# willis-richard/connect4

Measured on AMD Instinct MI355X. Metric: mcts_node_expansions_per_sec, higher is better.
Workload: dtype f32x3

## Files before the change

### connect4_amd/csrc/c4_engine.hip

```cpp
#include <hip/hip_runtime.h>
#include <hip/hip_fp16.h>
#include <hip/hip_bfloat16.h>

#include <algorithm>
#include <cmath>
#include <cstdarg>
#include <cstdio>
#include <cstdlib>
#include <cstring>
#include <limits>
#include <vector>

#include "../../include/c4_engine.h"
#include "c4_board.h"
#include "c4_net_dev.h"

#ifndef C4_DEADLINE_EVERY
#define C4_DEADLINE_EVERY 1
#endif
#ifndef C4_TERMQ
#define C4_TERMQ 1
#endif
#ifndef C4_FUSED_NET_STAMPS
#define C4_FUSED_NET_STAMPS 0
#endif
#ifndef C4_ASM_PICK
#define C4_ASM_PICK 1
#endif
#ifndef C4_SPECULATE
#define C4_SPECULATE 1
#endif
#ifndef C4_SPLIT_PHASES
#define C4_SPLIT_PHASES 0
#endif
#ifndef C4_DIV_NORMAL
#define C4_DIV_NORMAL 1
#endif
#ifndef C4_SCORE_ALL
#define C4_SCORE_ALL 1
#endif
#ifndef C4_PATH_ALL_LANES
#define C4_PATH_ALL_LANES 1
#endif
#ifndef C4_PEEL_BACKUP
#define C4_PEEL_BACKUP 1
#endif
#ifndef C4_NO_SUSPEND
#define C4_NO_SUSPEND 1
#endif
#ifndef C4_NET_SANITISES
#define C4_NET_SANITISES 1
#endif
#ifndef C4_WAIT_CLOCK_LAZY
#define C4_WAIT_CLOCK_LAZY 1
#endif
#ifndef C4_SPLIT_PAIRS
#define C4_SPLIT_PAIRS 1
#endif
#ifndef C4_SORT_SLOTS
#define C4_SORT_SLOTS 1
#endif
#ifndef C4_FILLERS
#define C4_FILLERS (C4_ORIENTED_Q && C4_SCORE_ALL)
#endif
#ifndef C4_VGPR_BASES
#define C4_VGPR_BASES 1
#endif
#ifndef C4_ORIENTED_Q
#define C4_ORIENTED_Q 1
#endif
#ifndef C4_COOP_LEGAL
#define C4_COOP_LEGAL 1
#endif
#ifndef C4_PICK_BPERM
#define C4_PICK_BPERM 1
#endif
#ifndef C4_EARLY_REQUEST
#define C4_EARLY_REQUEST 1
#endif

namespace {

using namespace c4;

constexpr int GROUP = 8;
constexpr int SLOTS_PER_BLOCK = 8;
constexpr int BLOCK = GROUP * SLOTS_PER_BLOCK;
constexpr int MAX_DEPTH = 44;

constexpr int SLOT_ACTIVE = 0;
constexpr int SLOT_PARKED = 1;
constexpr int SLOT_MOVE_DONE = 2;

__host__ __device__ __forceinline__ uint32_t pack_info(uint32_t base, uint32_t nchild, uint32_t status,
                                                       uint32_t bit, uint32_t pf64)
{
    return (base >> 3) | (nchild << 19) | (status << 22) | (bit << 25) | (pf64 << 31);
}
__host__ __device__ __forceinline__ uint32_t info_base(uint32_t i) { return (i & 0x7ffffu) << 3; }
__host__ __device__ __forceinline__ uint32_t info_nchild(uint32_t i) { return (i >> 19) & 7u; }
__host__ __device__ __forceinline__ uint32_t info_status(uint32_t i) { return (i >> 22) & 7u; }
__host__ __device__ __forceinline__ uint32_t info_bit(uint32_t i) { return (i >> 25) & 63u; }
__host__ __device__ __forceinline__ uint32_t info_move(uint32_t i) { return info_bit(i) / 7u; }
__host__ __device__ __forceinline__ uint32_t info_pf64(uint32_t i) { return i >> 31; }

struct __attribute__((aligned(16))) PathEntry {
    uint32_t node;
    uint32_t n;
    double w;
};

constexpr int BLOCK_BYTES = 256;
struct __attribute__((aligned(32))) Rec {
    double w;
    double q;
    double p;
// ... 112 lines not shown
__device__ __forceinline__ float lds_ldf(const float *p) { return *(lds_vf32_t *)p; }
__device__ __forceinline__ void lds_st64(uint64_t *p, uint64_t v) { *(lds_vu64_t *)p = v; }

__device__ __forceinline__ void group_fence()
{
    __builtin_amdgcn_fence(__ATOMIC_RELEASE, "workgroup");
    __builtin_amdgcn_fence(__ATOMIC_ACQUIRE, "workgroup");
}

__device__ __forceinline__ void philox_round(uint32_t c[4], const uint32_t k[2])
{
    const uint64_t p0 = (uint64_t)0xD2511F53u * c[0];
    const uint64_t p1 = (uint64_t)0xCD9E8D57u * c[2];
    const uint32_t n0 = (uint32_t)(p1 >> 32) ^ c[1] ^ k[0];
    const uint32_t n1 = (uint32_t)p1;
    const uint32_t n2 = (uint32_t)(p0 >> 32) ^ c[3] ^ k[1];
    const uint32_t n3 = (uint32_t)p0;
    c[0] = n0; c[1] = n1; c[2] = n2; c[3] = n3;
}
__device__ inline void philox4x32(uint32_t c[4], uint64_t seed)
{
    uint32_t k[2] = {(uint32_t)seed, (uint32_t)(seed >> 32)};
#pragma unroll
    for (int r = 0; r < 10; ++r) {
        philox_round(c, k);
        k[0] += 0x9E3779B9u;
        k[1] += 0xBB67AE85u;
    }
}
__device__ inline void rng_uniform2(uint64_t seed, long long gid, uint32_t ply, uint32_t stream, uint32_t idx,
                                    double &u0, double &u1)
{
    uint32_t c[4] = {(uint32_t)gid, (uint32_t)((uint64_t)gid >> 32), ply * 64u + stream, idx};
    philox4x32(c, seed);
    u0 = (double)((((uint64_t)c[0] << 32) | c[1]) >> 11) * (1.0 / 9007199254740992.0);
    u1 = (double)((((uint64_t)c[2] << 32) | c[3]) >> 11) * (1.0 / 9007199254740992.0);
}
__device__ inline double rng_gamma(uint64_t seed, long long gid, uint32_t ply, uint32_t stream, double alpha)
{
    double u0, u1;
    rng_uniform2(seed, gid, ply, stream, 0, u0, u1);
    double boost = 1.0;
    if (alpha < 1.0) {
        boost = pow(u0 > 0.0 ? u0 : 1e-300, 1.0 / alpha);
        alpha += 1.0;
    }
    const double dd = alpha - 1.0 / 3.0, cc = 1.0 / sqrt(9.0 * dd);
    for (uint32_t it = 1; it <= 24; ++it) {
        double a, b, uu, unused;
        rng_uniform2(seed, gid, ply, stream, 2 * it, a, b);
        rng_uniform2(seed, gid, ply, stream, 2 * it + 1, uu, unused);
        const double x = sqrt(-2.0 * log(a > 0.0 ? a : 1e-300)) * cos(6.283185307179586 * b);
        double v = 1.0 + cc * x;
        if (v <= 0.0) continue;
        v = v * v * v;
        if (uu < 1.0 - 0.0331 * x * x * x * x) return boost * dd * v;
        if (log(uu > 0.0 ? uu : 1e-300) < 0.5 * x * x + dd * (1.0 - v + log(v))) return boost * dd * v;
    }
    return boost * dd;
}

__device__ __forceinline__ double child_value_for(uint32_t status, uint32_t n, double q, int side)
{
    const bool term = status >= ST_XWIN;
#if C4_TERMQ
    const double v = q;
#else
    const double v = term ? 0.5 * (double)(status - ST_XWIN) : q;
#endif
    const double sv = side == 0 ? v : 1.0 - v;
    return (term || n > 0) ? sv : 0.0;
}

__device__ __forceinline__ double orient_q(double v, int parent_side)
{
#if C4_ORIENTED_Q
    return (parent_side & 1) ? 1.0 - v : v;
#else
    (void)parent_side;
    return v;
#endif
}

__device__ __forceinline__ double div_normal(double a, double b)
{
#if C4_DIV_NORMAL
    double r = __builtin_amdgcn_rcp(b);
    double e = __builtin_fma(-b, r, 1.0);
    r = __builtin_fma(r, e, r);
    e = __builtin_fma(-b, r, 1.0);
    r = __builtin_fma(r, e, r);
    const double q = a * r;
    const double rem = __builtin_fma(-b, q, a);
    return __builtin_fma(rem, r, q);
#else
    return a / b;
#endif
}

__device__ __forceinline__ double ucb_score(double A, double B, uint32_t nc, double p, double V, uint32_t pf64)
{
    const double pbc = A * div_normal(B, (double)(nc + 1));
    const double prior_score64 = pbc * p;
    const double s64 = prior_score64 + V;
    const float prior_score32 = (float)pbc * (float)p;
    const float s32 = prior_score32 + (float)V;
    return pf64 ? s64 : (double)s32;
}

__device__ __forceinline__ int legal_mask_group(uint64_t occ)
{
#if C4_COOP_LEGAL
    const int lane = (int)(threadIdx.x & (GROUP - 1));
    const bool legal = lane < WIDTH && col_count(occ, lane < WIDTH ? lane : 0) < HEIGHT;
    const unsigned long long b = __builtin_amdgcn_ballot_w64(legal);
    return (int)((b >> (threadIdx.x & 63u & ~(uint32_t)(GROUP - 1))) & 0x7fu);
#else
    return legal_mask(occ);
#endif
}

__device__ __forceinline__ int group_argmax(double s, int k)
{
#pragma unroll
    for (int m = 1; m < GROUP; m <<= 1) {
        const double os = __shfl_xor(s, m, GROUP);
        const int ok = __shfl_xor(k, m, GROUP);
        if (os > s || (os == s && ok > k)) { s = os; k = ok; }
    }
    return k;
}

template <int CTRL>
__device__ __forceinline__ uint32_t dpp_u32(uint32_t v)
{
    return (uint32_t)__builtin_amdgcn_update_dpp(0, (int)v, CTRL, 0xF, 0xF, true);
}
template <int CTRL>
__device__ __forceinline__ double dpp_f64(double v)
{
    const uint64_t b = (uint64_t)__double_as_longlong(v);
    const uint64_t r = ((uint64_t)dpp_u32<CTRL>((uint32_t)(b >> 32)) << 32) | dpp_u32<CTRL>((uint32_t)b);
    return __longlong_as_double((long long)r);
}
struct Pick {
    double s;
    int k;
    uint32_t n, info;
    double w;
};
#define C4_DPP_SELECT(CTRL)                                                                              \
    asm volatile("s_mov_b64 vcc, %[m]\n"                                                                 \
                 "s_nop 0\n"                                                                             \
                 "v_cndmask_b32_dpp %[n], %[n], %[n], vcc " CTRL " row_mask:0xf bank_mask:0xf\n"         \
                 "v_cndmask_b32_dpp %[i], %[i], %[i], vcc " CTRL " row_mask:0xf bank_mask:0xf\n"         \
                 "v_cndmask_b32_dpp %[wl], %[wl], %[wl], vcc " CTRL " row_mask:0xf bank_mask:0xf\n"      \
                 "v_cndmask_b32_dpp %[wh], %[wh], %[wh], vcc " CTRL " row_mask:0xf bank_mask:0xf\n"      \
                 : [n] "+v"(n), [i] "+v"(info), [wl] "+v"(wl), [wh] "+v"(wh)                              \
                 : [m] "s"(m)                                                                             \
                 : "vcc")
#if C4_ASM_PICK
#define C4_PICK_SELECT(CTRL)                                                                             \
    asm volatile("s_mov_b64 vcc, %[m]\n"                                                                 \
                 "s_nop 0\n"                                                                             \
                 "v_cndmask_b32 %[sl], %[ol], %[sl], vcc\n"                                               \
                 "v_cndmask_b32 %[sh], %[oh], %[sh], vcc\n"                                               \
                 "v_cndmask_b32_dpp %[n], %[n], %[n], vcc " CTRL " row_mask:0xf bank_mask:0xf\n"          \
                 "v_cndmask_b32_dpp %[i], %[i], %[i], vcc " CTRL " row_mask:0xf bank_mask:0xf\n"          \
                 "v_cndmask_b32_dpp %[wl], %[wl], %[wl], vcc " CTRL " row_mask:0xf bank_mask:0xf\n"       \
                 "v_cndmask_b32_dpp %[wh], %[wh], %[wh], vcc " CTRL " row_mask:0xf bank_mask:0xf\n"       \
                 : [sl] "+v"(sl), [sh] "+v"(sh), [n] "+v"(n), [i] "+v"(info), [wl] "+v"(wl), [wh] "+v"(wh) \
                 : [m] "s"(m), [ol] "v"(ol), [oh] "v"(oh)                                                   \
                 : "vcc")
template <int CTRL>
__device__ __forceinline__ void pick_step(double &s, uint32_t &n, uint32_t &info, uint32_t &wl, uint32_t &wh)
{
    const uint64_t sb = (uint64_t)__double_as_longlong(s);
    uint32_t sl = (uint32_t)sb, sh = (uint32_t)(sb >> 32);
    const uint32_t ol = dpp_u32<CTRL>(sl), oh = dpp_u32<CTRL>(sh);
    const double os = __longlong_as_double((long long)(((uint64_t)oh << 32) | ol));
    constexpr unsigned long long HIGH = CTRL == 0xB1 ? 0xAAAAAAAAAAAAAAAAull : (CTRL == 0x4E ? 0xCCCCCCCCCCCCCCCCull : 0xF0F0F0F0F0F0F0F0ull);
// ... 67 lines not shown
__device__ __forceinline__ double dirichlet_from_gamma(double nz, bool legal)
{
    if (!legal) nz = 0.0;
    double s = 0.0;
#pragma unroll
    for (int i = 0; i < 7; ++i) s = s + gshfl(nz, i);
    return nz / s;
}

__device__ __forceinline__ int sample_child_sq(double V, bool act, uint32_t nc, double u, int lane)
{
    const double w2 = act ? V * V : 0.0;
    double s2 = 0.0;
#pragma unroll
    for (int i = 0; i < 7; ++i) s2 = s2 + gshfl(w2, i);
    if (!(s2 > 0.0)) return -1;
    const double pk = w2 / s2;
    double acc = 0.0, cdf = 0.0;
#pragma unroll
    for (int i = 0; i < 7; ++i) {
        acc = acc + gshfl(pk, i);
        if (i == lane) cdf = acc;
    }
    const double last = gshfl(cdf, (int)nc - 1);
    cdf = cdf / last;
    const unsigned long long bal = __ballot(act && cdf <= u);
    const int cnt = __popcll((bal >> (((threadIdx.x & 63) / GROUP) * GROUP)) & 0xffull);
    return cnt < (int)nc ? cnt : (int)nc - 1;
}

template <class DevT>
__device__ __forceinline__ void publish_game(DevT &d, int g, long long gid, int len, int32_t result, int lane)
{
    group_fence();
    int ok = 0;
    unsigned long long t = 0;
    if (lane == 0) {
        const unsigned long long tail = *(volatile unsigned long long *)d.cold->ring_tail;
        unsigned long long old = *(volatile unsigned long long *)d.cold->ring_head;
        for (;;) {
            if (old - tail >= (unsigned long long)d.rec_cap) { atomicAdd(d.cold->dropped, 1ULL); break; }
            const unsigned long long seen = atomicCAS(d.cold->ring_head, old, old + 1);
            if (seen == old) { ok = 1; t = old; break; }
            old = seen;
        }
    }
    ok = gshfl(ok, 0);
    if (!ok) return;
    t = ((unsigned long long)gshfl((uint32_t)(t >> 32), 0) << 32) | gshfl((uint32_t)t, 0);
    c4_game_record *row = d.cold->ring + (size_t)(t % (unsigned long long)d.rec_cap);
    const size_t s0 = (size_t)g * 42;
    for (int i = lane; i < len; i += GROUP) {
        row->color0[i] = d.cold->stg_c0[s0 + i];
        row->color1[i] = d.cold->stg_c1[s0 + i];
        row->move[i] = d.cold->stg_move[s0 + i];
        row->value[i] = d.cold->stg_value[s0 + i];
    }
    double *rp = &row->policy[0][0];
    for (int i = lane; i < len * 7; i += GROUP) rp[i] = d.cold->stg_policy[s0 * 7 + i];
    if (lane == 0) { row->game_id = gid; row->length = len; row->result = result; }
}

__device__ __forceinline__ uint64_t group_xor64(uint64_t v)
{
    uint32_t lo = (uint32_t)v, hi = (uint32_t)(v >> 32);
    lo ^= dpp_u32<0xB1>(lo); hi ^= dpp_u32<0xB1>(hi);
    lo ^= dpp_u32<0x4E>(lo); hi ^= dpp_u32<0x4E>(hi);
    lo ^= dpp_u32<0x141>(lo); hi ^= dpp_u32<0x141>(hi);
    return ((uint64_t)hi << 32) | lo;
}
__device__ __forceinline__ uint64_t cache_key(uint64_t c0, uint64_t c1) { return c0 + (c0 | c1); }
template <class DevT>
__device__ __forceinline__ CacheEntry *cache_slot(DevT &d, uint64_t key)
{
    return d.cache + ((key * 0x9E3779B97F4A7C15ULL) >> (64 - d.cache_bits));
}
__device__ __forceinline__ uint64_t cache_check(uint64_t key, float value, float prior_lane, int lane)
{
    const uint32_t bits = lane < 7 ? __float_as_uint(prior_lane) : __float_as_uint(value);
    const uint64_t w = ((uint64_t)bits << 32) | (uint32_t)(bits * 0x9E3779B1u + (uint32_t)lane);
    const int r = (lane * 7 + 3) & 63;
    return key ^ group_xor64((w << r) | (w >> ((64 - r) & 63)));
}
template <class DevT>
__device__ __forceinline__ bool cache_probe(DevT &d, uint64_t c0, uint64_t c1, int lane, float &value, float &prior_lane)
{
    const uint64_t key = cache_key(c0, c1);
    const CacheEntry *e = cache_slot(d, key);
    const uint64_t k = e->key, chk = e->check;
    value = e->value;
    prior_lane = lane < 7 ? e->prior[lane] : 0.0f;
    return k == key && chk == cache_check(key, value, prior_lane, lane);
}
template <class DevT>
__device__ __forceinline__ void cache_insert(DevT &d, uint64_t c0, uint64_t c1, int lane, float value, float prior_lane)
{
    const uint64_t key = cache_key(c0, c1);
    CacheEntry *e = cache_slot(d, key);
    const uint64_t chk = cache_check(key, value, prior_lane, lane);
    if (lane < 7) e->prior[lane] = prior_lane;
    if (lane == 0) { e->value = value; e->check = chk; e->key = key; }
}

template <typename T>
__device__ __forceinline__ void store_plane(void *planes, size_t idx, float v);
template <> __device__ __forceinline__ void store_plane<float>(void *p, size_t i, float v) { ((float *)p)[i] = v; }
template <> __device__ __forceinline__ void store_plane<__half>(void *p, size_t i, float v) { ((__half *)p)[i] = __float2half(v); }
template <> __device__ __forceinline__ void store_plane<hip_bfloat16>(void *p, size_t i, float v) { ((hip_bfloat16 *)p)[i] = hip_bfloat16(v); }

constexpr uint32_t REQ_IDLE = 0, REQ_POSTED = 1, REQ_TAKEN = 2, REQ_ANSWERED = 3;
template <int EVAL, bool STAMPS = true, bool LDS_STATE = false, bool WAVE_SYNC = false, bool PATH_KEPT = false, class DevT = const Dev,
          bool SPLIT = false>
__device__ __forceinline__ void tree_step(DevT &d, const int g, const int lane, const int gl,
                                          PathEntry (*s_path)[MAX_DEPTH], Rec (*s_l1)[GROUP],
                                          const void *__restrict__ values_in,
                                          const void *__restrict__ priors_in, void *__restrict__ planes_out,
                                          uint64_t *leaf_out, SlotMem *sm = nullptr, const int ai_lds = 0,
                                          uint32_t *wg_stats = nullptr, const unsigned long long deadline = 0,
                                          uint32_t *req = nullptr, const int diag_stride = 0)
{
    (void)diag_stride;
    static_assert(!SPLIT || (WAVE_SYNC && LDS_STATE && PATH_KEPT), "the split kernel keeps slot states and paths in LDS");
    if (leaf_out && lane < 2) leaf_out[lane] = 0;
    if (g >= d.slot_hi) return;
    if (LDS_STATE) {
        if (sm->state() != SLOT_ACTIVE) {
            if (lane == 0) sm->flags = SlotMem::pack(sm->state(), 0, sm->need_root());
            return;
        }
    } else if (d.state[g] != SLOT_ACTIVE) {
        if (lane == 0) d.has_leaf[g] = 0;
        return;
    }
    constexpr bool SCORE_F32 = (EVAL == C4_EVAL_EXTERNAL_F32);
    const int ai = LDS_STATE ? ai_lds : g;

    const Pool pool{d.pool + (size_t)g * d.cap * (BLOCK_BYTES / 8)};
    PathEntry *gpath = d.path + (size_t)g * MAX_DEPTH;

    uint64_t root0, root1;
    uint32_t sims, nalloc, pdepth, pinfo, ply;
    int32_t pend, need_root;
    long long gid;
    if (LDS_STATE) {
        root0 = sm->root0; root1 = sm->root1;
        sims = sm->sims; nalloc = sm->nalloc; pend = sm->pend; pdepth = sm->pdepth; pinfo = sm->pinfo;
        need_root = sm->need_root(); ply = sm->ply; gid = sm->gid;
    } else {
        root0 = d.root_c0[g]; root1 = d.root_c1[g];
        sims = d.sims_done[g]; nalloc = d.n_alloc[g]; pend = d.pending[g]; pdepth = d.pending_depth[g];
        pinfo = d.pending_info[g]; need_root = d.need_root[g]; ply = d.ply[g]; gid = d.game_id[g];
    }
    double root_w = LDS_STATE ? sm->root_w : 0.0;
    int state = SLOT_ACTIVE;
    int has_leaf = 0;
    struct { uint32_t sims, expansions, children, terminal_sims, leaf_evals, depth_sum, moves, games_started,
                      games_finished, capped, cache_hits, cache_probes, bad_evals, spec_evals; } st = {};
    static_assert(sizeof(st) == N_STATS * 4, "launch-local stats mirror SlotStats");

    uint64_t leaf0 = 0, leaf1 = 0;
    double ev_value = 0.0, ev_prior = 0.0;
    bool apply_now = false;
    bool path_lds = (EVAL == C4_EVAL_CENTRE) || PATH_KEPT;
    bool fresh_eval = false;
    bool cached_answer = false;
    if (SPLIT && pend >= 0) {
        if (lds_ld(req) != REQ_ANSWERED) return;
        if (lane == 0) lds_st(req, REQ_IDLE);
    }
    if (pend >= 0) {
        leaf0 = LDS_STATE ? sm->leaf0 : d.leaf_c0[g];
        leaf1 = LDS_STATE ? sm->leaf1 : d.leaf_c1[g];
        if (EVAL == C4_EVAL_EXTERNAL_F32) {
            ev_value = (double)((const float *)values_in)[ai];
            ev_prior = lane < 7 ? (double)((const float *)priors_in)[(size_t)ai * 7 + lane] : 0.0;
        } else if (EVAL == C4_EVAL_EXTERNAL_F64) {
            ev_value = ((const double *)values_in)[ai];
            ev_prior = lane < 7 ? ((const double *)priors_in)[(size_t)ai * 7 + lane] : 0.0;
        }
        apply_now = true;
        fresh_eval = (EVAL == C4_EVAL_EXTERNAL_F32) && d.cache != nullptr;
    }

    auto stamp = [&](int i) {
        if (STAMPS && d.has_stamps && blockIdx.x < 256 && threadIdx.x == 0) d.cold->stamps[blockIdx.x * 8 + i] = __builtin_amdgcn_s_memtime();
    };
    stamp(0);
    asm volatile("s_waitcnt vmcnt(0)" ::: "memory");
    stamp(1);
    int levels_left = d.level_budget > 0 ? d.level_budget : 0x7fffffff;
    const unsigned long long t_begin = (!WAVE_SYNC && d.time_budget > 0) ? __builtin_amdgcn_s_memtime() : 0;
    bool resume = !(WAVE_SYNC && C4_NO_SUSPEND) && (pend == -2);
    bool l1_valid = false;
    int inner = 0;
    const unsigned long long wave_mask0 = WAVE_SYNC ? __builtin_amdgcn_ballot_w64(true) : 0ull;
    bool waiting = false;
#if C4_SPLIT_PHASES
    unsigned long long ph_t0 = 0, ph_iter = 0, ph_wait = 0, ph_apply = 0, ph_levels = 0, ph_n = 0, ph_ta = 0, ph_probe = 0, ph_term = 0;
    bool ph_was_waiting = false;
#endif
    for (;;) {
#if C4_SPLIT_PHASES
        if (SPLIT) { const unsigned long long tn = __builtin_amdgcn_s_memtime(); if (ph_t0) { (ph_was_waiting ? ph_wait : ph_iter) += tn - ph_t0; ph_n += ph_was_waiting ? 0 : 1; } ph_t0 = tn; ph_was_waiting = waiting; }
#endif
        if (SPLIT) {
#if C4_WAIT_CLOCK_LAZY
            if (__builtin_amdgcn_ballot_w64(!waiting) == 0) {
                __builtin_amdgcn_s_sleep(4);
                if ((long long)(__builtin_amdgcn_s_memtime() - deadline) > 0) { has_leaf = 1; break; }
            }
            if (waiting) {
#else
            if (__builtin_amdgcn_ballot_w64(!waiting) == 0) __builtin_amdgcn_s_sleep(4);
            if (waiting) {
                if ((long long)(__builtin_amdgcn_s_memtime() - deadline) > 0) { has_leaf = 1; break; }
#endif
                if (lds_ld(req) != REQ_ANSWERED) continue;
#if C4_SPLIT_PHASES
                if (lane == 0) {
                    uint32_t *sums = req - ai + 3 * diag_stride;
                    atomicAdd(&sums[2], ((uint32_t)__builtin_amdgcn_s_memtime() - lds_ld(req + 2 * diag_stride)) >> 6);
                }
#endif
                ev_value = (double)lds_ldf((const float *)values_in + ai);
                ev_prior = lane < 7 ? (double)lds_ldf((const float *)priors_in + (size_t)ai * 7 + lane) : 0.0;
                if (lane == 0) lds_st(req, REQ_IDLE);
                waiting = false;
                apply_now = true;
                fresh_eval = d.cache != nullptr;
            }
        }
        if (apply_now) {
#if C4_SPLIT_PHASES
            ph_ta = __builtin_amdgcn_s_memtime();
#endif
            apply_now = false;
            if (!(SPLIT && C4_NET_SANITISES) && !cached_answer) {
                const bool bad = !(ev_value >= 0.0 && ev_value <= 1.0) || !(ev_prior >= 0.0 && ev_prior <= 3.0e38);
                if (__ballot(bad) >> (((threadIdx.x & 63) / GROUP) * GROUP) & 0xffull) {
                    if (!(ev_value >= 0.0 && ev_value <= 1.0)) ev_value = 0.5;
                    if (!(ev_prior >= 0.0 && ev_prior <= 3.0e38)) ev_prior = 0.0;
                    st.bad_evals += 1;
                }
            }
            if (fresh_eval) {
                fresh_eval = false;
                cache_insert(d, leaf0, leaf1, lane, (float)ev_value, (float)ev_prior);
            }
            cached_answer = false;
            const uint64_t occ = leaf0 | leaf1;
            const int age = popc64(occ);
            const int mask = legal_mask_group(occ);
            const bool legal = lane < 7 && ((mask >> lane) & 1);
            double prn;
            uint32_t pf64;
            if (SCORE_F32) {
                const float pf = legal ? (float)ev_prior : 0.0f;
                float s = 0.0f;
#if C4_COOP_LEGAL
                float pall[7];
#pragma unroll
                for (int i = 0; i < 7; ++i) pall[i] = gshfl(pf, i);
#pragma unroll
                for (int i = 0; i < 7; ++i) s = s + pall[i];
#else
#pragma unroll
                for (int i = 0; i < 7; ++i) s = s + gshfl(pf, i);
#endif
                prn = s > 0.0f ? (double)(pf / s) : (legal ? 1.0 / (double)__popc(mask) : 0.0);
                pf64 = 0;
            } else {
                const double pd = legal ? ev_prior : 0.0;
                double s = 0.0;
#pragma unroll
                for (int i = 0; i < 7; ++i) s = s + gshfl(pd, i);
                prn = s > 0.0 ? pd / s : (legal ? 1.0 / (double)__popc(mask) : 0.0);
                pf64 = 1;
            }
            if (pdepth == 0 && d.use_noise) {
                double nz = 0.0;
                if (lane < 7) {
                    if (d.rng_tape) nz = (gid < d.cold->tape_games) ? d.cold->noise_tape[((size_t)gid * 42 + ply) * 7 + lane] : 0.0;
                    else nz = rng_gamma(d.seed, gid, ply, (uint32_t)lane, d.alpha);
                }
                nz = dirichlet_from_gamma(nz, legal);
                const double keep = 1.0 - d.frac;
                const double a = SCORE_F32 ? (double)((float)prn * (float)keep) : prn * keep;
                const double b = nz * d.frac;
                prn = a + b;
                pf64 = 1;
            }
            const uint32_t nchild = (uint32_t)__popc(mask);
            const uint32_t base = nalloc * GROUP;
            nalloc += 1;
#if C4_FILLERS
            {
                const int below = (1 << lane) - 1;
                Rec nr{0.0, -std::numeric_limits<double>::infinity(), 0.0, 0u, pack_info(0, 0, ST_FRESH, 0, 0)};
                uint32_t k = nchild + (uint32_t)__popc(~mask & 0x7f & below);
                if (legal) {
                    k = (uint32_t)__popc(mask & below);
                    uint64_t c0 = leaf0, c1 = leaf1;
                    const uint32_t bit = (uint32_t)(H1 * lane + col_count(occ, lane));
                    const uint32_t cst = make_move(c0, c1, lane);
                    nr = Rec{0.0, cst >= ST_XWIN ? orient_q(0.5 * (double)(cst - ST_XWIN), age) : 0.0, prn, 0u, pack_info(0, 0, cst, bit, 0)};
                }
                *pool.rec(base + k) = nr;
            }
#else
            if (legal) {
                const uint32_t k = (uint32_t)__popc(mask & ((1 << lane) - 1));
                uint64_t c0 = leaf0, c1 = leaf1;
                const uint32_t bit = (uint32_t)(H1 * lane + col_count(occ, lane));
                const uint32_t cst = make_move(c0, c1, lane);
                const uint32_t idx = base + k;
                *pool.rec(idx) = Rec{0.0, cst >= ST_XWIN ? orient_q(0.5 * (double)(cst - ST_XWIN), age) : 0.0, prn, 0u, pack_info(0, 0, cst, bit, 0)};
            }
#endif
            if (lane == 0) {
                if (l1_valid && pdepth == 1) {
                    Rec &c = s_l1[gl][pend & 7];
                    c.n = 1;
                    c.w = ev_value;
                    c.q = orient_q(ev_value, age - 1);
                    c.info = pack_info(base, nchild, ST_EVALUATED, info_bit(pinfo), pf64);
                }
                pool.n(pend) = 1;
                pool.w(pend) = ev_value;
                pool.q(pend) = orient_q(ev_value, age - 1);
                pool.info(pend) = pack_info(base, nchild, ST_EVALUATED, info_bit(pinfo), pf64);
            }
            {
                auto back_up = [&](uint32_t i) {
                    const PathEntry e = path_lds ? s_path[gl][i] : gpath[i];
                    const double nw = e.w + ev_value, nq = orient_q(div_normal(nw, (double)(e.n + 1)), age + (int)pdepth + (int)i + 1);
                    pool.n(e.node) = e.n + 1;
                    pool.w(e.node) = nw;
                    pool.q(e.node) = nq;
                    if (l1_valid && i == 1) { Rec &c = s_l1[gl][e.node & 7]; c.n = e.n + 1; c.w = nw; c.q = nq; }
                };
#if C4_PEEL_BACKUP
                if ((uint32_t)lane < pdepth) back_up((uint32_t)lane);
                for (uint32_t i = lane + GROUP; i < pdepth; i += GROUP) back_up(i);
#else
                for (uint32_t i = lane; i < pdepth; i += GROUP) back_up(i);
#endif
            }
            root_w = pdepth == 0 ? ev_value : root_w + ev_value;
            if (pdepth == 0) l1_valid = false;
            st.leaf_evals += 1;
            st.children += nchild;
            if (pdepth > 0) sims += 1;
            (void)age;
            pend = -1;
            group_fence();
            stamp(2);
#if C4_SPLIT_PHASES
            ph_apply += __builtin_amdgcn_s_memtime() - ph_ta;
#endif
        }

        if (need_root) {
            need_root = 0;
            l1_valid = false;
            nalloc = 1;
            sims = 0;
            pend = 0;
            pdepth = 0;
            pinfo = pack_info(0, 0, ST_FRESH, 0, 0);
            leaf0 = root0;
            leaf1 = root1;
            if (EVAL == C4_EVAL_CENTRE) {
                ev_value = centre_value(leaf0, leaf1);
                ev_prior = 1.0 / 7.0;
                apply_now = true;
                continue;
            }
            if (EVAL == C4_EVAL_EXTERNAL_F32 && d.cache) {
                float cv, cp;
                st.cache_probes += 1;
                if (cache_probe(d, leaf0, leaf1, lane, cv, cp)) {
                    st.cache_hits += 1;
                    ev_value = (double)cv;
                    ev_prior = (double)cp;
                    apply_now = true;
                    cached_answer = true;
                    continue;
                }
            }
            if (SPLIT) {
                if (lane == 0) {
                    lds_st64(&sm->leaf0, leaf0);
                    lds_st64(&sm->leaf1, leaf1);
#if C4_SPLIT_PHASES
                    lds_st(req + diag_stride, (uint32_t)__builtin_amdgcn_s_memtime());
#endif
                    lds_st(req, REQ_POSTED);
                }
                waiting = true;
                continue;
            }
            has_leaf = 1;
            break;
        }

        if (sims >= (uint32_t)d.S) {
            const uint32_t rinfo = pool.info(0);
            const uint32_t cb = info_base(rinfo), nc = info_nchild(rinfo);
            const bool act = lane < (int)nc;
            const uint32_t cn = act ? pool.n(cb + lane) : 0;
            const double cq = act ? pool.q(cb + lane) : 0.0;
            const uint32_t ci = act ? pool.info(cb + lane) : 0;
            const int root_age = popc64(root0 | root1);
            const int side = root_age & 1;
            const double V = act ? (C4_ORIENTED_Q ? cq : child_value_for(info_status(ci), cn, cq, side)) : 0.0;
            double vs = 0.0;
#pragma unroll
            for (int i = 0; i < 7; ++i) vs = vs + gshfl(V, i);
            const double pol = act ? (vs == 0.0 ? 1.0 / (double)nc : V / vs) : 0.0;
            int kb = -1;
            double u = -1.0;
            if (root_age < d.nsm) {
                if (d.rng_tape) u = (gid < d.cold->tape_games) ? d.cold->u_tape[(size_t)gid * 42 + ply] : -1.0;
                else { double u1; rng_uniform2(d.seed, gid, ply, 32u, 0, u, u1); }
            }
            if (u >= 0.0) kb = sample_child_sq(V, act, nc, u, lane);
            if (kb < 0) kb = group_argmax(act ? V : -1.0, act ? lane : -1);
            const uint32_t bi = gshfl(ci, kb);
            const uint32_t bn = gshfl(cn, kb);
#if C4_ORIENTED_Q
            const double cw = act ? pool.w(cb + lane) : 0.0;
            const double bq = div_normal(gshfl(cw, kb), (double)(bn > 0 ? bn : 1u));
#else
            const double bq = gshfl(cq, kb);
#endif
            const int mv = (int)info_move(bi);
// ... 207 lines not shown
            const uint32_t cb = info_base(cinfo), nc = info_nchild(cinfo), pf64 = info_pf64(cinfo);
            if (cN == 1) st.expansions += 1;
            const bool act = lane < (int)nc;
            const uint32_t idx = cb + lane;
            const double2 ab = d.tabAB[cN];
            asm volatile("" ::: "memory");
            Rec r = {};
            if (depth == 0 && l1_valid) {
                if (act) r = s_l1[gl][lane];
            } else {
                if (act) r = *pool.rec(idx);
                if (depth == 0) {
                    if (act) s_l1[gl][lane] = r;
                    l1_valid = true;
                }
            }
            const uint32_t n = r.n, inf = r.info;
            const double w = r.w, q = r.q, p = r.p;
            const double A = ab.x, B = ab.y;
            if (STAMPS && d.has_stamps) {
                asm volatile("s_waitcnt vmcnt(0)" ::: "memory");
                const unsigned long long t1 = __builtin_amdgcn_s_memtime();
                lvl_wait += t1 - lvl_t0;
                lvl_t0 = t1;
            }
            const double V = C4_ORIENTED_Q ? q : child_value_for(info_status(inf), n, q, age & 1);
            const double s = act ? ucb_score(A, B, n, p, V, pf64) : -std::numeric_limits<double>::infinity();
            Pick best{s, act ? lane : -1, n, inf, w};
            group_pick(best);
            cN = best.n;
            cW = best.w;
            cinfo = best.info;
            cur = cb + (uint32_t)best.k;
            {
                const uint64_t stone = 1ULL << info_bit(cinfo);
                b0 ^= (age & 1) ? 0ULL : stone;
                b1 ^= (age & 1) ? stone : 0ULL;
            }
            age += 1;
            depth += 1;
            if (lane == 0) s_path[gl][depth] = PathEntry{cur, cN, cW};
            if (STAMPS && d.has_stamps) {
                const unsigned long long t2 = __builtin_amdgcn_s_memtime();
                lvl_alu += t2 - lvl_t0;
                lvl_t0 = t2;
                lvl_cnt += 1;
            }
        }
#endif
        if (STAMPS && d.has_stamps && blockIdx.x < 256 && threadIdx.x == 0) {
            d.cold->stamps[blockIdx.x * 8 + 7] = (lvl_wait << 32) | (lvl_alu & 0xffffffffu);
            d.cold->stamps[blockIdx.x * 8 + 6] = ((unsigned long long)lvl_cnt << 32) | depth;
        }
        if (!(WAVE_SYNC && C4_NO_SUSPEND) && info_status(cinfo) == ST_EVALUATED) {
            lds_fence();
            for (uint32_t i = lane; i <= depth; i += GROUP) gpath[i] = s_path[gl][i];
            if (lane == 0) {
                d.cold->cont_cur[g] = cur;
                d.cold->cont_n[g] = cN;
                d.cold->cont_w[g] = cW;
                if (LDS_STATE) { sm->leaf0 = b0; sm->leaf1 = b1; }
                else { d.leaf_c0[g] = b0; d.leaf_c1[g] = b1; }
            }
            pend = -2;
            pdepth = depth;
            pinfo = cinfo;
            break;
        }
#if C4_SPLIT_PHASES
        ph_levels += __builtin_amdgcn_s_memtime() - ph_tl;
#endif
        st.depth_sum += depth;
        stamp(3);
        const uint32_t lst = info_status(cinfo);
        if (lst >= ST_XWIN) {
#if C4_SPLIT_PHASES
            const unsigned long long ph_tt = __builtin_amdgcn_s_memtime();
#endif
            const double value = 0.5 * (double)(lst - ST_XWIN);
            lds_fence();
            {
                auto back_up = [&](uint32_t i) {
                    const PathEntry e = s_path[gl][i];
                    const double nw = e.w + value, nq = orient_q(div_normal(nw, (double)(e.n + 1)), age + (int)depth + (int)i + 1);
                    pool.n(e.node) = e.n + 1;
                    pool.w(e.node) = nw;
                    pool.q(e.node) = nq;
                    if (l1_valid && i == 1) { Rec &c = s_l1[gl][e.node & 7]; c.n = e.n + 1; c.w = nw; c.q = nq; }
                };
#if C4_PEEL_BACKUP
                if ((uint32_t)lane <= depth) back_up((uint32_t)lane);
                for (uint32_t i = lane + GROUP; i <= depth; i += GROUP) back_up(i);
#else
                for (uint32_t i = lane; i <= depth; i += GROUP) back_up(i);
#endif
            }
            root_w = root_w + value;
            sims += 1;
            st.sims += 1;
            st.terminal_sims += 1;
            group_fence();
#if C4_SPLIT_PHASES
            ph_term += __builtin_amdgcn_s_memtime() - ph_tt;
#endif
            continue;
        }
        pend = (int32_t)cur;
        pdepth = depth;
        pinfo = cinfo;
        leaf0 = b0;
        leaf1 = b1;
        st.sims += 1;
        if (EVAL == C4_EVAL_CENTRE) {
            ev_value = centre_value(b0, b1);
            ev_prior = 1.0 / 7.0;
            lds_fence();
            apply_now = true;
            continue;
        }
        lds_fence();
        if (EVAL == C4_EVAL_EXTERNAL_F32 && d.cache) {
            float cv, cp;
            st.cache_probes += 1;
#if C4_SPLIT_PHASES
            const unsigned long long ph_tp = __builtin_amdgcn_s_memtime();
            const bool ph_hit = cache_probe(d, b0, b1, lane, cv, cp);
            asm volatile("s_waitcnt vmcnt(0)" ::: "memory");
            ph_probe += __builtin_amdgcn_s_memtime() - ph_tp;
            if (ph_hit) {
#else
            if (cache_probe(d, b0, b1, lane, cv, cp)) {
#endif
                st.cache_hits += 1;
                ev_value = (double)cv;
                ev_prior = (double)cp;
                path_lds = true;
                apply_now = true;
                cached_answer = true;
                continue;
            }
        }
        if (!PATH_KEPT)
            for (uint32_t i = lane; i < depth; i += GROUP) gpath[i] = s_path[gl][i];
        if (SPLIT) {
            if (lane == 0) {
                lds_st64(&sm->leaf0, leaf0);
                lds_st64(&sm->leaf1, leaf1);
#if C4_SPLIT_PHASES
                lds_st(req + diag_stride, (uint32_t)__builtin_amdgcn_s_memtime());
#endif
                lds_st(req, REQ_POSTED);
            }
            waiting = true;
            continue;
        }
        has_leaf = 1;
        break;
    }

    stamp(4);
    if (has_leaf) {
        if (lane == 0) {
            if (LDS_STATE) { sm->leaf0 = leaf0; sm->leaf1 = leaf1; }
            else { d.leaf_c0[g] = leaf0; d.leaf_c1[g] = leaf1; }
        }
        if (leaf_out && lane == 0) { leaf_out[0] = leaf0; leaf_out[1] = leaf1; }
        if (planes_out) {
            const int o_to_move = (popc64(leaf0 | leaf1) & 1) ? 0 : 1;
            const size_t pb = (size_t)g * 126;
            for (int e = lane; e < 126; e += GROUP) {
                const float v = plane_element(leaf0, leaf1, o_to_move, e);
                if (d.planes_dtype == C4_PLANES_F32) store_plane<float>(planes_out, pb + e, v);
                else if (d.planes_dtype == C4_PLANES_F16) store_plane<__half>(planes_out, pb + e, v);
                else store_plane<hip_bfloat16>(planes_out, pb + e, v);
            }
        }
    }
    if (LDS_STATE) {
        if (lane == 0) {
            sm->root_w = root_w;
            sm->root0 = root0;
            sm->root1 = root1;
            sm->sims = sims;
            sm->nalloc = nalloc;
            sm->pend = (has_leaf || pend == -2) ? pend : -1;
            sm->pdepth = pdepth;
            sm->pinfo = pinfo;
            sm->ply = ply;
            sm->gid = gid;
            sm->flags = SlotMem::pack(state, has_leaf, need_root);
#if C4_SPLIT_PHASES
            if (SPLIT && d.has_stamps && g < 256) { unsigned long long *o = d.cold->stamps + (size_t)g * 8; o[0] = ph_iter; o[1] = ph_wait; o[2] = ph_apply; o[3] = ph_levels; o[4] = ph_n; o[5] = ph_probe; o[6] = ph_term; }
#endif
            const uint32_t *sv = (const uint32_t *)&st;
#pragma unroll
            for (int i = 0; i < N_STATS; ++i)
                if (sv[i]) atomicAdd(&wg_stats[i], sv[i]);
        }
        return;
    }
    if (lane == 0) {
        d.has_leaf[g] = has_leaf;
        d.root_c0[g] = root0;
        d.root_c1[g] = root1;
        d.sims_done[g] = sims;
        d.n_alloc[g] = nalloc;
        d.pending[g] = (has_leaf || pend == -2) ? pend : -1;
        d.pending_depth[g] = pdepth;
        d.pending_info[g] = pinfo;
        d.need_root[g] = need_root;
        d.ply[g] = ply;
        d.game_id[g] = gid;
        d.state[g] = state;
        uint64_t *sp = d.stats + (size_t)g * N_STATS;
        const uint32_t *sv = (const uint32_t *)&st;
#pragma unroll
        for (int i = 0; i < N_STATS; ++i) sp[i] += sv[i];
    }
    asm volatile("s_waitcnt vmcnt(0)" ::: "memory");
    stamp(5);
}

template <int EVAL>
__global__ __launch_bounds__(BLOCK) void c4_step_kernel(Dev d, const void *__restrict__ values_in,
                                                        const void *__restrict__ priors_in,
                                                        void *__restrict__ planes_out)
{
    __shared__ PathEntry s_path[SLOTS_PER_BLOCK][MAX_DEPTH];
    __shared__ Rec s_l1[SLOTS_PER_BLOCK][GROUP];
    const int lane = threadIdx.x & (GROUP - 1);
    const int gl = threadIdx.x / GROUP;
    const int g = d.slot_lo + blockIdx.x * SLOTS_PER_BLOCK + gl;
    tree_step<EVAL>(d, g, lane, gl, s_path, s_l1, values_in, priors_in, planes_out, nullptr);
}

template <int TS>
__global__ __launch_bounds__(c4net::NTHREADS) void c4_selfplay_kernel(Dev d, c4net::NetDev nd, float *__restrict__ values,
                                                                      float *__restrict__ priors, int n_steps)
{
    using namespace c4net;
    static_assert(TS % NWAVES == 0 && TS % P == 0 && TS <= 64, "slots per workgroup");
    __shared__ __attribute__((aligned(16))) _Float16 act[2][(ROWS + 1) * CS];
    __shared__ __attribute__((aligned(16))) half8 wbuf[2][WCHUNKS];
    __shared__ __attribute__((aligned(16))) float4 mlp[MLP_F4];
    __shared__ uint64_t sleaf[2][TS];
    __shared__ int smap[TS];
    __shared__ int sn;
    __shared__ SlotMem smem[TS];
    __shared__ float s_val[TS];
    __shared__ float s_pri[TS * 7];
    __shared__ uint32_t s_stats[N_STATS];
    static_assert((sizeof(PathEntry) * MAX_DEPTH + sizeof(Rec) * GROUP) * TS <= sizeof(_Float16) * ROWS * CS, "tree-phase LDS must fit the activation buffer");
    PathEntry (*s_path)[MAX_DEPTH] = reinterpret_cast<PathEntry (*)[MAX_DEPTH]>(&act[0][0]);
    Rec (*s_l1)[GROUP] = reinterpret_cast<Rec (*)[GROUP]>(&act[0][0] + sizeof(PathEntry) * MAX_DEPTH * TS / sizeof(_Float16));
    const int slot0 = blockIdx.x * TS;
    const int wv = threadIdx.x >> 6;
    if (threadIdx.x < TS) {
        const int p = threadIdx.x, g = slot0 + p;
        SlotMem m = {};
        m.flags = SlotMem::pack(SLOT_PARKED, 0, 0);
        if (g < d.G) {
            m.root0 = d.root_c0[g]; m.root1 = d.root_c1[g]; m.leaf0 = d.leaf_c0[g]; m.leaf1 = d.leaf_c1[g];
            m.gid = d.game_id[g]; m.sims = d.sims_done[g]; m.nalloc = d.n_alloc[g]; m.pend = d.pending[g];
            m.pdepth = d.pending_depth[g]; m.pinfo = d.pending_info[g];
            m.ply = d.ply[g]; m.flags = SlotMem::pack(d.state[g], d.has_leaf[g], d.need_root[g]);
            m.root_w = *(const double *)(d.pool + (size_t)g * d.cap * (BLOCK_BYTES / 8));
        }
        smem[p] = m;
    }
    if (threadIdx.x < N_STATS) s_stats[threadIdx.x] = 0;
    for (int i = threadIdx.x; i < TS * 8; i += NTHREADS) {
        const int p = i >> 3, k = i & 7;
        const bool ok = slot0 + p < d.G;
        if (k == 7) s_val[p] = ok ? values[slot0 + p] : 0.0f;
        else s_pri[p * 7 + k] = ok ? priors[(size_t)(slot0 + p) * 7 + k] : 0.0f;
// ... 1526 lines not shown
```

Before: 278.9 million.

## Precompute child expansion and backup state in the shadow of cache probe loads

Splits the cache probe into issue and resolve steps. In split mode, the child-move generation (legal mask, move status, terminal q) and the backup reciprocal prep are computed between the two, while the global loads are still in flight. The results are packed into a register word and reused when the evaluation is applied. This hides probe latency and shortens the apply phase, but adds register pressure and bit-packing complexity, and the work is wasted when the probe hits the cache.

```diff
diff --git a/connect4_amd/csrc/c4_engine.hip b/connect4_amd/csrc/c4_engine.hip
--- a/connect4_amd/csrc/c4_engine.hip
+++ b/connect4_amd/csrc/c4_engine.hip
@@ -32,6 +32,9 @@
 #endif
 #ifndef C4_SPLIT_PHASES
 #define C4_SPLIT_PHASES 0
+#endif
+#ifndef C4_APPLY_SHADOW
+#define C4_APPLY_SHADOW 1
 #endif
 #ifndef C4_DIV_NORMAL
 #define C4_DIV_NORMAL 1
@@ -310,7 +313,7 @@
 #endif
 }
 
-__device__ __forceinline__ double div_normal(double a, double b)
+__device__ __forceinline__ double div_prepare(double b)
 {
 #if C4_DIV_NORMAL
     double r = __builtin_amdgcn_rcp(b);
@@ -318,13 +321,24 @@
     r = __builtin_fma(r, e, r);
     e = __builtin_fma(-b, r, 1.0);
     r = __builtin_fma(r, e, r);
+    return r;
+#else
+    (void)b;
+    return 0.0;
+#endif
+}
+__device__ __forceinline__ double div_finish(double a, double b, double r)
+{
+#if C4_DIV_NORMAL
     const double q = a * r;
     const double rem = __builtin_fma(-b, q, a);
     return __builtin_fma(rem, r, q);
 #else
+    (void)r;
     return a / b;
 #endif
 }
+__device__ __forceinline__ double div_normal(double a, double b) { return div_finish(a, b, div_prepare(b)); }
 
 __device__ __forceinline__ double ucb_score(double A, double B, uint32_t nc, double p, double V, uint32_t pf64)
 {
@@ -558,15 +572,32 @@
     const int r = (lane * 7 + 3) & 63;
     return key ^ group_xor64((w << r) | (w >> ((64 - r) & 63)));
 }
+struct CacheProbe {
+    uint64_t key, k, chk;
+    float value, prior_lane;
+};
+template <class DevT>
+__device__ __forceinline__ CacheProbe cache_probe_issue(DevT &d, uint64_t c0, uint64_t c1, int lane)
+{
+    CacheProbe p;
+    p.key = cache_key(c0, c1);
+    const CacheEntry *e = cache_slot(d, p.key);
+    p.k = e->key;
+    p.chk = e->check;
+    p.value = e->value;
+    p.prior_lane = e->prior[lane < 7 ? lane : 0];
+    return p;
+}
+__device__ __forceinline__ bool cache_probe_resolve(const CacheProbe &p, int lane, float &value, float &prior_lane)
+{
+    value = p.value;
+    prior_lane = lane < 7 ? p.prior_lane : 0.0f;
+    return p.k == p.key && p.chk == cache_check(p.key, value, prior_lane, lane);
+}
 template <class DevT>
 __device__ __forceinline__ bool cache_probe(DevT &d, uint64_t c0, uint64_t c1, int lane, float &value, float &prior_lane)
 {
-    const uint64_t key = cache_key(c0, c1);
-    const CacheEntry *e = cache_slot(d, key);
-    const uint64_t k = e->key, chk = e->check;
-    value = e->value;
-    prior_lane = lane < 7 ? e->prior[lane] : 0.0f;
-    return k == key && chk == cache_check(key, value, prior_lane, lane);
+    return cache_probe_resolve(cache_probe_issue(d, c0, c1, lane), lane, value, prior_lane);
 }
 template <class DevT>
 __device__ __forceinline__ void cache_insert(DevT &d, uint64_t c0, uint64_t c1, int lane, float value, float prior_lane)
@@ -671,8 +702,47 @@
     int inner = 0;
     const unsigned long long wave_mask0 = WAVE_SYNC ? __builtin_amdgcn_ballot_w64(true) : 0ull;
     bool waiting = false;
+    constexpr uint32_t XP_VALID = 1u, XP_LEGAL = 2u, XP_BACKUP = 1u << 21, XP_INFO = 0x7fc00000u;
+    uint32_t xp = 0, xb_node = 0, xb_n1 = 0;
+    double xb_w = 0.0, xb_b = 0.0, xb_r = 0.0;
+    auto prepare_children = [&]() {
+        const uint64_t occ = leaf0 | leaf1;
+        const int age = popc64(occ);
+        const int mask = legal_mask_group(occ);
+        const bool legal = lane < 7 && ((mask >> lane) & 1);
+        const int below = (1 << lane) - 1;
+        uint32_t k = (uint32_t)__popc(mask) + (uint32_t)__popc(~mask & 0x7f & below);
+        uint32_t ci = pack_info(0, 0, ST_FRESH, 0, 0);
+        double tq = 0.0;
+        if (legal) {
+            k = (uint32_t)__popc(mask & below);
+            uint64_t c0 = leaf0, c1 = leaf1;
+            const uint32_t bit = (uint32_t)(H1 * lane + col_count(occ, lane));
+            const uint32_t cst = make_move(c0, c1, lane);
+            tq = cst >= ST_XWIN ? orient_q(0.5 * (double)(cst - ST_XWIN), age) : 0.0;
+            ci = pack_info(0, 0, cst, bit, 0);
+        }
+        const uint32_t tq_hi = (uint32_t)((unsigned long long)__double_as_longlong(tq) >> 32);
+        xp = (xp & XP_BACKUP) | XP_VALID | (legal ? XP_LEGAL : 0u) | (k << 2) | ((uint32_t)mask << 5) | ((uint32_t)age << 12) |
+             ((((uint32_t)age + pdepth + (uint32_t)lane + 1u) & 1u) << 18) | (((tq_hi >> 20) & 3u) << 19) | ci;
+    };
+    auto prepare_backup = [&](const bool in_lds) {
+#if C4_PEEL_BACKUP
+        if ((uint32_t)lane < pdepth) {
+            const PathEntry e = in_lds ? s_path[gl][lane] : gpath[lane];
+            xb_node = e.node;
+            xb_n1 = e.n + 1;
+            xb_w = e.w;
+            xb_b = (double)(e.n + 1);
+            xb_r = div_prepare(xb_b);
+        }
+#else
+        (void)in_lds;
+#endif
+        xp |= XP_BACKUP;
+    };
 #if C4_SPLIT_PHASES
-    unsigned long long ph_t0 = 0, ph_iter = 0, ph_wait = 0, ph_apply = 0, ph_levels = 0, ph_n = 0, ph_ta = 0, ph_probe = 0, ph_term = 0;
+    unsigned long long ph_t0 = 0, ph_iter = 0, ph_wait = 0, ph_apply = 0, ph_levels = 0, ph_n = 0, ph_ta = 0, ph_probe = 0, ph_term = 0, ph_shadow = 0;
     bool ph_was_waiting = false;
 #endif
     for (;;) {
@@ -724,10 +794,13 @@
                 cache_insert(d, leaf0, leaf1, lane, (float)ev_value, (float)ev_prior);
             }
             cached_answer = false;
-            const uint64_t occ = leaf0 | leaf1;
-            const int age = popc64(occ);
-            const int mask = legal_mask_group(occ);
-            const bool legal = lane < 7 && ((mask >> lane) & 1);
+            if (!(xp & XP_VALID)) prepare_children();
+            if (!(xp & XP_BACKUP)) prepare_backup(path_lds);
+            const uint32_t xw = xp;
+            xp = 0;
+            const int age = (int)((xw >> 12) & 63u);
+            const int mask = (int)((xw >> 5) & 0x7fu);
+            const bool legal = (xw & XP_LEGAL) != 0;
             double prn;
             uint32_t pf64;
             if (SCORE_F32) {
@@ -771,26 +844,15 @@
             nalloc += 1;
 #if C4_FILLERS
             {
-                const int below = (1 << lane) - 1;
-                Rec nr{0.0, -std::numeric_limits<double>::infinity(), 0.0, 0u, pack_info(0, 0, ST_FRESH, 0, 0)};
-                uint32_t k = nchild + (uint32_t)__popc(~mask & 0x7f & below);
-                if (legal) {
-                    k = (uint32_t)__popc(mask & below);
-                    uint64_t c0 = leaf0, c1 = leaf1;
-                    const uint32_t bit = (uint32_t)(H1 * lane + col_count(occ, lane));
-                    const uint32_t cst = make_move(c0, c1, lane);
-                    nr = Rec{0.0, cst >= ST_XWIN ? orient_q(0.5 * (double)(cst - ST_XWIN), age) : 0.0, prn, 0u, pack_info(0, 0, cst, bit, 0)};
-                }
-                *pool.rec(base + k) = nr;
+                const uint32_t tc = (xw >> 19) & 3u;
+                const uint32_t q_hi = legal ? (tc ? 0x3fc00000u | (tc << 20) : 0u) : 0xfff00000u;
+                *pool.rec(base + ((xw >> 2) & 7u)) = Rec{0.0, __longlong_as_double((long long)((unsigned long long)q_hi << 32)), legal ? prn : 0.0, 0u, xw & XP_INFO};
             }
 #else
             if (legal) {
-                const uint32_t k = (uint32_t)__popc(mask & ((1 << lane) - 1));
-                uint64_t c0 = leaf0, c1 = leaf1;
-                const uint32_t bit = (uint32_t)(H1 * lane + col_count(occ, lane));
-                const uint32_t cst = make_move(c0, c1, lane);
-                const uint32_t idx = base + k;
-                *pool.rec(idx) = Rec{0.0, cst >= ST_XWIN ? orient_q(0.5 * (double)(cst - ST_XWIN), age) : 0.0, prn, 0u, pack_info(0, 0, cst, bit, 0)};
+                const uint32_t tc = (xw >> 19) & 3u;
+                const uint32_t q_hi = tc ? 0x3fc00000u | (tc << 20) : 0u;
+                *pool.rec(base + ((xw >> 2) & 7u)) = Rec{0.0, __longlong_as_double((long long)((unsigned long long)q_hi << 32)), prn, 0u, xw & XP_INFO};
             }
 #endif
             if (lane == 0) {
@@ -816,7 +878,13 @@
                     if (l1_valid && i == 1) { Rec &c = s_l1[gl][e.node & 7]; c.n = e.n + 1; c.w = nw; c.q = nq; }
                 };
 #if C4_PEEL_BACKUP
-                if ((uint32_t)lane < pdepth) back_up((uint32_t)lane);
+                if ((uint32_t)lane < pdepth) {
+                    const double nw = xb_w + ev_value, nq = orient_q(div_finish(nw, xb_b, xb_r), (int)((xw >> 18) & 1u));
+                    pool.n(xb_node) = xb_n1;
+                    pool.w(xb_node) = nw;
+                    pool.q(xb_node) = nq;
+                    if (l1_valid && lane == 1) { Rec &c = s_l1[gl][xb_node & 7]; c.n = xb_n1; c.w = nw; c.q = nq; }
+                }
                 for (uint32_t i = lane + GROUP; i < pdepth; i += GROUP) back_up(i);
 #else
                 for (uint32_t i = lane; i < pdepth; i += GROUP) back_up(i);
@@ -827,7 +895,6 @@
             st.leaf_evals += 1;
             st.children += nchild;
             if (pdepth > 0) sims += 1;
-            (void)age;
             pend = -1;
             group_fence();
             stamp(2);
@@ -1201,7 +1268,8 @@
             {
                 auto back_up = [&](uint32_t i) {
                     const PathEntry e = s_path[gl][i];
-                    const double nw = e.w + value, nq = orient_q(div_normal(nw, (double)(e.n + 1)), age + (int)depth + (int)i + 1);
+                    const double b = (double)(e.n + 1);
+                    const double nw = e.w + value, nq = orient_q(div_finish(nw, b, div_prepare(b)), age + (int)depth + (int)i + 1);
                     pool.n(e.node) = e.n + 1;
                     pool.w(e.node) = nw;
                     pool.q(e.node) = nq;
@@ -1243,13 +1311,28 @@
             st.cache_probes += 1;
 #if C4_SPLIT_PHASES
             const unsigned long long ph_tp = __builtin_amdgcn_s_memtime();
-            const bool ph_hit = cache_probe(d, b0, b1, lane, cv, cp);
+#endif
+            CacheProbe probe = cache_probe_issue(d, b0, b1, lane);
+#if C4_APPLY_SHADOW
+            if (SPLIT) {
+                asm volatile("" : "+v"(leaf0), "+v"(leaf1) : : "memory");
+#if C4_SPLIT_PHASES
+                const unsigned long long ph_ts = __builtin_amdgcn_s_memtime();
+#endif
+                prepare_children();
+                prepare_backup(true);
+                asm volatile("" : "+v"(xp), "+v"(xb_r));
+#if C4_SPLIT_PHASES
+                ph_shadow += __builtin_amdgcn_s_memtime() - ph_ts;
+#endif
+                asm volatile("" : "+v"(probe.k), "+v"(probe.chk), "+v"(probe.value), "+v"(probe.prior_lane));
+            }
+#endif
+#if C4_SPLIT_PHASES
             asm volatile("s_waitcnt vmcnt(0)" ::: "memory");
             ph_probe += __builtin_amdgcn_s_memtime() - ph_tp;
-            if (ph_hit) {
-#else
-            if (cache_probe(d, b0, b1, lane, cv, cp)) {
-#endif
+#endif
+            if (cache_probe_resolve(probe, lane, cv, cp)) {
                 st.cache_hits += 1;
                 ev_value = (double)cv;
                 ev_prior = (double)cp;
@@ -1309,7 +1392,7 @@
             sm->gid = gid;
             sm->flags = SlotMem::pack(state, has_leaf, need_root);
 #if C4_SPLIT_PHASES
-            if (SPLIT && d.has_stamps && g < 256) { unsigned long long *o = d.cold->stamps + (size_t)g * 8; o[0] = ph_iter; o[1] = ph_wait; o[2] = ph_apply; o[3] = ph_levels; o[4] = ph_n; o[5] = ph_probe; o[6] = ph_term; }
+            if (SPLIT && d.has_stamps && g < 256) { unsigned long long *o = d.cold->stamps + (size_t)g * 8; o[0] = ph_iter; o[1] = ph_wait; o[2] = ph_apply; o[3] = ph_levels; o[4] = ph_n; o[5] = ph_probe; o[6] = ph_term; o[7] = ph_shadow; }
 #endif
             const uint32_t *sv = (const uint32_t *)&st;
 #pragma unroll
```

Result: faster. 281.8 million, median of 6 (+1.1%).
